# AdrianPerezHerrero/HDP-GPC

Measured on AMD Instinct MI355X. Metric: GP log-lik evals/sec (NxK batch, T-point segments), higher is better.
Workload: dtype f64; 1 GPU; BASELINE configs[1]: synthetic 2048 segments x 8 clusters, T=128, fp64, irregular segment grids (per-pair Gram + Cholesky + score); segments=2048, segments_per_gpu=2048, clusters=8, T=128

## Files before the change

hdpgpc_amd/csrc/hgp_internal.hpp:

```cpp
#pragma once
#include <hip/hip_runtime.h>
#include <stdint.h>
#include <stdlib.h>

#include <vector>

#include "../../include/hdpgpc_hip.h"

constexpr int WAVES = 4;

static inline int launch_status() {
  hipError_t e = hipGetLastError();
  return e == hipSuccess ? 0 : 1000 + (int)e;
}

static inline int nb_for(int n) {
  int nb = (n + 15) / 16;
  nb = (nb + 1) & ~1;
  return nb < 2 ? 2 : nb;
}

static inline bool env_on(const char* name) {
  const char* v = getenv(name);
  return v && v[0] && v[0] != '0';
}

constexpr double PAIRS_CUT = 55.45177444479562;
constexpr int PAIRS_FB_CAP = 65536;

static inline int acc_grid_for(int nb) { return nb > 8 ? 256 : 512; }

struct hgp_pairs_plan {
  int T, K, TP, NB;
  std::vector<double> theta;
  std::vector<int32_t> perm;
  std::vector<int> grp_beg, grp_end;
  std::vector<double> grp_ell;
  double *d_theta, *d_scal, *d_A, *d_S, *d_Z, *d_Kinv, *d_P, *d_Q, *d_Mp, *d_ap, *d_xb;
  int32_t* d_perm;
  bool coop = false;
  double* d_escr = nullptr;
  int32_t* d_eflags = nullptr;
  int nscr = 0;
  long escr_stride = 0;
  double acc_tol = 1e-9;
  double* d_Lop = nullptr;
  double* d_LTop = nullptr;
  double* d_Dop = nullptr;
  double* d_Sop = nullptr;
  double* d_mu = nullptr;
  int32_t* d_acc_list = nullptr;
  double* d_sscr = nullptr;
  int32_t* d_fb = nullptr;
  int score_out = 0;
};

int hgp_internal_acc_prep(hgp_pairs_plan* p, const double* mean, hipStream_t st);
int hgp_internal_pairs_acc(const hgp_pairs_plan* p, const double* x, const double* y, int N, int Ts, const double* first_noise,
                           const int32_t* sel, double* out_quad, double* out_logdet, int32_t* out_info, hipStream_t st);
size_t hgp_internal_acc_bytes(int TP, int K, size_t* sizes );

int hgp_internal_loglik_rows_b(const double* q, int N, int K, int B, double* out, hipStream_t st);
int hgp_internal_assign_b(const double* fmsg, const double* bmsg, int N, int K, int B, int64_t* labels, double* last_log, hipStream_t st);
// ... 50 lines not shown
```

hdpgpc_amd/csrc/hgp_kernels.hip:

```cpp
#include <hip/hip_runtime.h>
#include <math.h>
#include <stdint.h>
#include <string.h>

#include <algorithm>
#include <mutex>
#include <new>
#include <vector>

#include "../../include/hdpgpc_hip.h"
#include "hgp_internal.hpp"
#include "tile_f64.hpp"

using namespace hgp;

namespace {

__global__ void k_gram_rbf(const double* __restrict__ x, int nx, const double* __restrict__ y, int ny, double c,
                           double ell, double noise, int one_arg, double* __restrict__ K) {
  size_t idx = (size_t)blockIdx.x * blockDim.x + threadIdx.x;
  if (idx >= (size_t)nx * ny) return;
  int i = (int)(idx / ny), j = (int)(idx % ny);
  double u = x[i] / ell - (one_arg ? x[j] : y[j]) / ell;
  double v = c * exp(-0.5 * (u * u));
  if (one_arg && i == j) v = c + noise;
  K[idx] = v;
}

__global__ void k_mfma_probe(const double* __restrict__ A, const double* __restrict__ B, double* __restrict__ C) {
  const int lane = threadIdx.x & 63, g = lane >> 4, c = lane & 15;
  d4 acc = (d4){0.0, 0.0, 0.0, 0.0};
#pragma unroll
  for (int s = 0; s < 4; ++s) acc = mfma(A[c * 16 + 4 * s + g], B[(4 * s + g) * 16 + c], acc);
// ... 44 lines not shown
    add_diag<NB>(U, a.jitter_rel * fmax(dm, F64_EPS), T, lane);
  }
  PivotAcc pa;
  pa.init();
  wave_factor<NB, 0>(U, R, scr, nullptr, nullptr, lane, pa, A, T, T);
#pragma unroll
  for (int I = 0; I < NB; ++I)
#pragma unroll
    for (int J = I + 1; J < NB; ++J) {
      const int ln = launder(lane);
#pragma unroll
      for (int r = 0; r < 4; ++r) {
        int i = 16 * I + (ln >> 4) + 4 * r, j = 16 * J + (ln & 15);
        if (i < T && j < T) A[(size_t)i * T + j] = 0.0;
      }
    }
  if (lane == 0) {
    if (a.info) a.info[m] = pa.info;
    if (a.logdet) a.logdet[m] = pa.logdet();
  }
}

template <int NB>
__global__ __launch_bounds__(64 * WAVES) void k_wave_inv(PotrfArgs a) {
  __shared__ __attribute__((aligned(16))) double scr_all[WAVES * DIAG_SCR];
  const int wave = threadIdx.x >> 6, lane = threadIdx.x & 63;
  const int g = lane >> 4, c = lane & 15;
  const int w = blockIdx.x * WAVES + wave;
  const int m = w / NB, Jc = w % NB;
  const int T = a.T;
  if (m >= a.b || 16 * Jc >= T) return;
  double* scr = scr_all + wave * DIAG_SCR;
  const double* A = a.A + (size_t)m * T * T;
  d4 U[NB * (NB + 1) / 2];
  d4 R[NB];
  if (a.symmetric) load_upper_only<NB>(U, A, T, T, lane);
  else if constexpr (NB <= 6) load_sym_upper_burst<NB>(U, A, T, T, lane, scr);
  else load_sym_upper<NB>(U, A, T, T, lane, scr);
  {
    double sh = a.add;
    if (a.jitter_rel != 0.0) sh += a.jitter_rel * fmax(diag_abs_mean<NB>(U, T, lane, a.add), F64_EPS);
    if (sh != 0.0) add_diag<NB>(U, sh, T, lane);
  }
#pragma unroll
  for (int K = 0; K < NB; ++K)
#pragma unroll
    for (int r = 0; r < 4; ++r) R[K][r] = (K == Jc && g + 4 * r == c) ? 1.0 : 0.0;
  PivotAcc pa;
  pa.init();
  wave_factor<NB, 1>(U, R, scr, nullptr, nullptr, lane, pa, nullptr, 0, T);
  double* Z = a.Linv + (size_t)m * T * T;
#pragma unroll
  for (int K = 0; K < NB; ++K)
#pragma unroll
    for (int r = 0; r < 4; ++r) {
      const int i = 16 * K + g + 4 * r, j = 16 * Jc + c;
      if (i < T && j < T) Z[(size_t)i * T + j] = (K >= Jc) ? R[K][r] : 0.0;
    }
  if (a.inv_info && Jc == 0 && lane == 0 && a.info) a.info[m] = pa.info;
}

template <int NB>
void launch_wave_inv(const PotrfArgs& a, hipStream_t st) {
  const int waves = a.b * NB;
  hipLaunchKernelGGL(k_wave_inv<NB>, dim3((waves + WAVES - 1) / WAVES), dim3(64 * WAVES), 0, st, a);
}

struct ScoreArgs {
  const double* Y;
  int ldy;
  const double* mean;
  long mean_stride;
  const double* Sigma;
  long sigma_stride;
  int T;
  int ld_sigma;
  const int32_t* item_mat;
  const int32_t* item_mean;
  const double* item_add;
  const int32_t* item_off;
  const int32_t* item_cnt;
  int n_items;
// ... 275 lines not shown
#pragma unroll
      for (int s = 0; s < 4; ++s) {
        const int row = 16 * I + c, col = 16 * I + 4 * s + g;
        wv[s] = (row < T && col < T) ? Z[(size_t)row * T + col] : ((row == col) ? 1.0 : 0.0);
      }
      d4 z = (d4){0.0, 0.0, 0.0, 0.0};
#pragma unroll
      for (int s = 0; s < 4; ++s) z = mfma_sub(wv[s], acc0[s], z);
      Zc[I] = z;
    }
  }
  const bool bad = info && info[m] != 0;
#pragma unroll
  for (int I = 0; I < NB; ++I) {
#pragma unroll
    for (int r = 0; r < 4; ++r) {
      const int row = 16 * I + g + 4 * r, col = 16 * Kc + c;
      if (row < T && col < T && I != Kc) Z[(size_t)row * T + col] = bad ? __builtin_nan("") : ((I > Kc) ? Zc[I][r] : 0.0);
    }
  }
}

template <int NB>
__global__ __launch_bounds__(64 * WAVES) void k_coop_inv(PotrfArgs a) {
  using C = Coop<NB>;
  extern __shared__ __attribute__((aligned(16))) double smem[];
  double* rowbuf = smem;
  double* Rbuf = rowbuf + NB * 256;
  double* Wbuf = Rbuf + NB * 256;
  double* scr = Wbuf + 256;
  double* red = scr + DIAG_SCR;
  const int wave = __builtin_amdgcn_readfirstlane(threadIdx.x >> 6), lane = threadIdx.x & 63;
  const int g = lane >> 4, c = lane & 15;
  const int m = blockIdx.x, Jc = blockIdx.y;
  const int T = a.T;
  if (16 * Jc >= T) return;
  const double* A = a.A + (size_t)m * T * T;
  d4 U[C::NT];
  coop_load_sym_upper<NB>(U, A, T, T, wave, lane, rowbuf + wave * DIAG_SCR);
  __syncthreads();
  {
    double sh = a.add;
    if (a.jitter_rel != 0.0) {
      const double dm = coop_diag_abs_mean<NB>(U, T, wave, lane, a.add, red);
      sh += a.jitter_rel * fmax(dm, F64_EPS);
    }
    if (sh != 0.0) coop_add_diag<NB>(U, sh, T, wave, lane);
  }
  for (int K = wave; K < NB; K += WAVES) {
    d4 v;
#pragma unroll
    for (int r = 0; r < 4; ++r) v[r] = (K == Jc && g + 4 * r == c) ? 1.0 : 0.0;
    lds_tile_store(Rbuf, K, lane, v);
  }
  __syncthreads();
  PivotAcc pa;
  pa.init();
  coop_factor<NB, true>(U, rowbuf, Rbuf, Wbuf, scr, wave, lane, pa, nullptr, 0, T);
  double* Z = a.Linv + (size_t)m * T * T;
  for (int K = wave; K < NB; K += WAVES) {
    const d4 z = lds_tile_load(Rbuf, K, lane);
#pragma unroll
    for (int r = 0; r < 4; ++r) {
      const int i = 16 * K + g + 4 * r, j = 16 * Jc + c;
      if (i < T && j < T) Z[(size_t)i * T + j] = (K >= Jc) ? z[r] : 0.0;
    }
  }
  if (a.inv_info && Jc == 0) {
    int info;
    (void)coop_logdet_info(pa, wave, lane, red, reinterpret_cast<int*>(red + 8), info);
    if (threadIdx.x == 0 && a.info) a.info[m] = info;
  }
}

}

int hgp_internal_ensure_dynamic_lds(const void* fn, size_t bytes) {
  static std::mutex mu;
  static std::vector<std::pair<const void*, int>> done;
  int dv = 0;
  if (hipGetDevice(&dv) != hipSuccess) return launch_status();
  std::lock_guard<std::mutex> lk(mu);
  for (const auto& d : done)
    if (d.first == fn && d.second == dv) return 0;
  const hipError_t e = hipFuncSetAttribute(fn, hipFuncAttributeMaxDynamicSharedMemorySize, (int)bytes);
  if (e != hipSuccess) return 1000 + (int)e;
  done.emplace_back(fn, dv);
  return 0;
}

namespace {

template <int NB>
int launch_coop_score(const ScoreArgs& a, hipStream_t st) {
  const size_t lds = sizeof(double) * Coop<NB>::LDS_DOUBLES;
// ... 22 lines not shown
  if (int rc_ = hgp_internal_ensure_dynamic_lds(reinterpret_cast<const void*>(&k_coop_inv<NB>), lds)) return rc_;
  hipLaunchKernelGGL(k_coop_inv<NB>, dim3(a.b, NB), dim3(64 * WAVES), lds, st, a);
  return launch_status();
}

struct GemmArgs {
  const double* A;
  const double* B;
  double* C;
  int M, N, Kd, lda, ldb, ldc;
  long sA, sB, sC;
  double alpha, beta;
  int tA, tB;
  int nb2 = 1;
  long sA2 = 0, sB2 = 0, sC2 = 0;
  const double* D = nullptr;
  int ldd = 0;
  long sD = 0;
  int boff = 0;
  int triA = 0;
};

template <int TRIP>
__global__ __launch_bounds__(64 * WAVES) void k_gemm(GemmArgs a) {
  const int wave = threadIdx.x >> 6, lane = threadIdx.x & 63;
  const int g = lane >> 4, c = lane & 15;
  const int ntn = (a.N + 15) / 16, ntm = (a.M + 15) / 16;
  const int tile = blockIdx.x * WAVES + wave;
  if (tile >= ntm * ntn) return;
  const int ti = tile / ntn, tj = tile % ntn;
  const int by = (int)blockIdx.y + a.boff;
  const int b1 = by / a.nb2, b2 = by % a.nb2;
  const double* A = a.A + (size_t)b1 * a.sA + (size_t)b2 * a.sA2;
  const double* B = a.B + (size_t)b1 * a.sB + (size_t)b2 * a.sB2;
  double* C = a.C + (size_t)b1 * a.sC + (size_t)b2 * a.sC2;
  d4 acc = (d4){0.0, 0.0, 0.0, 0.0};
  const int row = 16 * ti + c, col = 16 * tj + c;
  int nk = (a.Kd + 3) / 4;
  if (a.triA && !a.tA) nk = min(nk, 4 * (ti + 1));
  for (int k0 = 0; k0 < nk; k0 += TRIP) {
    double av[TRIP], bv[TRIP];
#pragma unroll
    for (int u = 0; u < TRIP; ++u) {
      const int k = 4 * (k0 + u) + g;
      av[u] = 0.0;
      bv[u] = 0.0;
      if (k < a.Kd) {
        if (row < a.M) av[u] = a.tA ? A[(size_t)k * a.lda + row] : A[(size_t)row * a.lda + k];
        if (col < a.N) bv[u] = a.tB ? B[(size_t)col * a.ldb + k] : B[(size_t)k * a.ldb + col];
      }
    }
#pragma unroll
    for (int u = 0; u < TRIP; ++u) acc = mfma(av[u], bv[u], acc);
  }
#pragma unroll
  for (int r = 0; r < 4; ++r) {
    const int i = 16 * ti + g + 4 * r;
    if (i < a.M && col < a.N) {
      double v = a.alpha * acc[r];
      if (a.beta != 0.0)
        v += a.beta * (a.D ? a.D[(size_t)b1 * a.sD + (size_t)i * a.ldd + col] : C[(size_t)i * a.ldc + col]);
      C[(size_t)i * a.ldc + col] = v;
    }
  }
}

__global__ __launch_bounds__(64 * WAVES) void k_gemm22(GemmArgs a) {
  const int wave = threadIdx.x >> 6, lane = threadIdx.x & 63;
  const int g = lane >> 4, c = lane & 15;
  const int ntn = a.N / 32, ntm = a.M / 32;
  const int tile = blockIdx.x * WAVES + wave;
  if (tile >= ntm * ntn) return;
  const int ti = tile / ntn, tj = tile % ntn;
  const int by = (int)blockIdx.y + a.boff;
  const int b1 = by / a.nb2, b2 = by % a.nb2;
  const double* A = a.A + (size_t)b1 * a.sA + (size_t)b2 * a.sA2 + (size_t)(32 * ti + c) * a.lda + g;
  const double* B = a.B + (size_t)b1 * a.sB + (size_t)b2 * a.sB2 + (size_t)g * a.ldb + 32 * tj + c;
  double* C = a.C + (size_t)b1 * a.sC + (size_t)b2 * a.sC2;
  d4 acc[2][2];
#pragma unroll
  for (int i = 0; i < 2; ++i)
#pragma unroll
    for (int j = 0; j < 2; ++j) acc[i][j] = (d4){0.0, 0.0, 0.0, 0.0};
  int nk = a.Kd / 4;
  if (a.triA) nk = min(nk, 8 * (ti + 1));
  constexpr int TR = 8;
  for (int k0 = 0; k0 < nk; k0 += TR) {
// ... 847 lines not shown
      const int oi = redi[tid + w];
      if (ov > red[tid] || (ov == red[tid] && oi < redi[tid])) {
        red[tid] = ov;
        redi[tid] = oi;
      }
    }
    __syncthreads();
  }
  if (tid == 0) first[t] = (any_nan || redi[0] >= K * K) ? 0 : redi[0];
}

struct PrepArgs {
  const double* xb;
  const double* mean;
  const double* Sigma;
  int T, TP, K;
  const double* theta;
  double* scal;
  double* A;
  double* S;
  double* xb_copy;
};

__global__ __launch_bounds__(256) void k_prep_build(PrepArgs a) {
  __shared__ double red[256];
  __shared__ int redi[256];
  const int k = blockIdx.x, tid = threadIdx.x;
  const int T = a.T, TP = a.TP;
  const double* Sg = a.Sigma + (size_t)k * T * T;
  const double c = a.theta[3 * k], ell = a.theta[3 * k + 1], noise = a.theta[3 * k + 2];
  double s_abs = 0.0, s_sgn = 0.0;
  for (int i = tid; i < T; i += 256) {
    double d = Sg[(size_t)i * T + i];
    s_abs += fabs(d);
    s_sgn += d;
  }
  red[tid] = s_abs;
  __syncthreads();
  for (int o = 128; o > 0; o >>= 1) {
    if (tid < o) red[tid] += red[tid + o];
    __syncthreads();
  }
  const double mean_abs = red[0] / T;
  __syncthreads();
  red[tid] = s_sgn;
  __syncthreads();
  for (int o = 128; o > 0; o >>= 1) {
    if (tid < o) red[tid] += red[tid + o];
    __syncthreads();
  }
  const double mS = red[0] / T;
  int bad = 0;
  for (int i = tid; i < T; i += 256) {
    double d = Sg[(size_t)i * T + i];
    if (!(fabs(d - mS) <= 1e-8 + 1e-5 * fabs(mS))) bad = 1;
  }
  redi[tid] = bad;
  __syncthreads();
  for (int o = 128; o > 0; o >>= 1) {
    if (tid < o) redi[tid] |= redi[tid + o];
    __syncthreads();
  }
  const double jit = 1e-4 * fmax(mean_abs, F64_EPS);
  if (tid == 0 && blockIdx.y == 0) {
    double* sc = a.scal + 8 * k;
    sc[0] = c;
    sc[1] = ell;
    sc[2] = noise;
    sc[3] = redi[0] ? 0.0 : 1.0;
    sc[4] = mS;
    sc[5] = jit;
    sc[6] = 0.0;
  }
  if (k == 0 && blockIdx.y == 0)
    for (int i = tid; i < TP; i += 256) a.xb_copy[i] = (i < T) ? a.xb[i] : 0.0;
  double* Ak = a.A + (size_t)k * TP * TP;
  double* Sk = a.S + (size_t)k * TP * TP;
  for (int idx = blockIdx.y * 256 + tid; idx < TP * TP; idx += gridDim.y * 256) {
    int i = idx / TP, j = idx % TP;
    double av, sv = 0.0;
    if (i < T && j < T) {
      double u = a.xb[i] / ell - a.xb[j] / ell;
      av = c * exp(-0.5 * (u * u));
      if (i == j) av += jit;
      sv = 0.5 * (Sg[(size_t)i * T + j] + Sg[(size_t)j * T + i]);
    } else {
      av = (i == j) ? 1.0 : 0.0;
    }
    Ak[idx] = av;
    Sk[idx] = sv;
  }
}

struct PrepFinalArgs {
  const double* Q;
  const double* Kinv;
  const double* mean;
  double* scal;
  int T, TP;
  double* Mp;
  double* ap;
  int interleave;
  int32_t* fb;
};

__global__ __launch_bounds__(256) void k_prep_final(PrepFinalArgs a) {
  const int k = blockIdx.x, tid = threadIdx.x;
  if (a.fb && k == 0 && blockIdx.y == 0 && tid == 0) {
    a.fb[0] = 0;
    a.fb[1 + PAIRS_FB_CAP] = 0;
  }
  const int T = a.T, TP = a.TP;
  const double c = a.scal[8 * k];
  const double* Q = a.Q + (size_t)k * TP * TP;
  const double* Ki = a.Kinv + (size_t)k * TP * TP;
  double* Mp = a.Mp + (size_t)k * TP * TP;
  __shared__ double tq[32][33], tk[32][33];
  const int NHh = (TP / 16) / 2, nt = TP / 32;
  const int tx = tid & 31, ty = tid >> 5;
  for (int t = blockIdx.y; t < nt * nt; t += gridDim.y) {
    const int bi = t / nt, bj = t % nt;
    __syncthreads();
#pragma unroll
    for (int r = 0; r < 4; ++r) {
      const int y = ty + 8 * r;
      tq[y][tx] = Q[(size_t)(32 * bj + y) * TP + 32 * bi + tx];
      tk[y][tx] = Ki[(size_t)(32 * bj + y) * TP + 32 * bi + tx];
    }
    __syncthreads();
#pragma unroll
    for (int r = 0; r < 4; ++r) {
      const int y = ty + 8 * r;
      const int i = 32 * bi + y, j = 32 * bj + tx;
      double v = 0.0;
      if (i < T && j < T)
        v = (c * c) * (0.5 * (Q[(size_t)i * TP + j] + tq[tx][y]) - 0.5 * (Ki[(size_t)i * TP + j] + tk[tx][y]));
      int jp = j;
      if (a.interleave) {
        const int hh = j / (16 * NHh), tl = (j / 16) % NHh, cc = j % 16;
        const int loc = (tl < 2 * (NHh / 2)) ? 32 * (tl / 2) + 2 * cc + (tl & 1) : 16 * (NHh - 1) + cc;
        jp = 16 * NHh * hh + loc;
      }
      Mp[(size_t)i * TP + jp] = v;
    }
  }
  const double* mu = a.mean + (size_t)k * T;
  __shared__ double red[256];
  double rmax = 0.0;
  for (int i = blockIdx.y * 256 + tid; i < TP; i += gridDim.y * 256) {
    double s = 0.0, rs = 0.0;
    if (i < T) {
#pragma unroll 8
      for (int j = 0; j < T; ++j) {
        const double kij = Ki[(size_t)j * TP + i];
        s = fma(kij, mu[j], s);
        rs += fabs(kij);
      }
    }
    a.ap[(size_t)k * TP + i] = c * s;
    rmax = fmax(rmax, rs);
  }
  red[tid] = rmax;
  __syncthreads();
  for (int o = 128; o > 0; o >>= 1) {
    if (tid < o) red[tid] = fmax(red[tid], red[tid + o]);
    __syncthreads();
  }
  if (tid == 0) atomicMax(reinterpret_cast<unsigned long long*>(a.scal + 8 * k + 6), (unsigned long long)__double_as_longlong(red[0]));
}

}

#ifdef HGP_STAMPS
unsigned long long* hgp_internal_stamp_dev = nullptr;
#endif

static int tp_for(int n) {
  if (n <= HGP_MAX_T_WAVE) return 16 * nb_for(n);
  return n <= 192 ? 192 : 256;
}

static size_t plan_bytes(int T, int Ts_max, int K, size_t* offs ) {
  const size_t TP = (size_t)tp_for(std::max(T, Ts_max));
  const size_t mat = (size_t)K * TP * TP * sizeof(double);
  size_t o = 0;
  auto take = [&](size_t bytes) {
    size_t at = o;
    o += (bytes + 255) & ~(size_t)255;
    return at;
  };
  size_t tmp[24] = {0};
// ... 97 lines not shown
  return launch_status();
}

size_t hgp_pairs_plan_device_bytes(int T, int Ts_max, int K) {
  if (T <= 0 || Ts_max <= 0 || K <= 0) return 0;
  return plan_bytes(T, Ts_max, K, nullptr);
}

int hgp_pairs_plan_create(hgp_pairs_plan** plan, int T, int Ts_max, int K, const double* theta_host, void* dev_buf,
                          size_t dev_bytes) {
  if (!plan || !theta_host || !dev_buf || T <= 0 || Ts_max <= 0 || K <= 0) return -1;
  if (T > HGP_MAX_T_COOP || Ts_max > HGP_MAX_T_COOP) return -2;
  size_t offs[24];
  if (dev_bytes < plan_bytes(T, Ts_max, K, offs)) return -1;
  for (int k = 0; k < K; ++k)
    if (!(theta_host[3 * k] > 0.0) || !(theta_host[3 * k + 1] > 0.0)) return -1;
  hgp_pairs_plan* p = new (std::nothrow) hgp_pairs_plan();
  if (!p) return -1;
  p->T = T;
  p->K = K;
  p->TP = tp_for(std::max(T, Ts_max));
  p->NB = p->TP / 16;
  p->coop = p->TP > HGP_MAX_T_WAVE;
  p->theta.assign(theta_host, theta_host + 3 * (size_t)K);
  p->perm.resize(K);
  for (int k = 0; k < K; ++k) p->perm[k] = k;
  std::stable_sort(p->perm.begin(), p->perm.end(),
                   [&](int a, int b) { return p->theta[3 * a + 1] < p->theta[3 * b + 1]; });
  for (int i = 0; i < K;) {
    int j = i;
    double ell = p->theta[3 * p->perm[i] + 1];
    while (j < K && p->theta[3 * p->perm[j] + 1] == ell) ++j;
    p->grp_beg.push_back(i);
    p->grp_end.push_back(j);
    p->grp_ell.push_back(ell);
    i = j;
  }
  char* base = (char*)dev_buf;
  p->d_theta = (double*)(base + offs[0]);
  p->d_scal = (double*)(base + offs[1]);
  p->d_A = (double*)(base + offs[2]);
  p->d_S = (double*)(base + offs[3]);
  p->d_Z = (double*)(base + offs[4]);
  p->d_Kinv = (double*)(base + offs[5]);
  p->d_P = (double*)(base + offs[6]);
  p->d_Q = (double*)(base + offs[7]);
// ... 24 lines not shown
      delete p;
      return 1000 + (int)hipGetLastError();
    }
  }
  if (hipMemcpy(p->d_theta, p->theta.data(), sizeof(double) * 3 * K, hipMemcpyHostToDevice) != hipSuccess ||
      hipMemcpy(p->d_perm, p->perm.data(), sizeof(int32_t) * K, hipMemcpyHostToDevice) != hipSuccess) {
    delete p;
    return 1000 + (int)hipGetLastError();
  }
  *plan = p;
  return 0;
}

void hgp_pairs_plan_destroy(hgp_pairs_plan* plan) { delete plan; }

const double* hgp_pairs_plan_scalars(const hgp_pairs_plan* plan) { return plan ? plan->d_scal : nullptr; }

int hgp_pairs_plan_update(hgp_pairs_plan* p, const double* x_basis, const double* mean, const double* Sigma,
                          int32_t* info, void* stream) {
  if (!p || !x_basis || !mean || !Sigma) return -1;
  hipStream_t st = (hipStream_t)stream;
  const int K = p->K, T = p->T, TP = p->TP;
  PrepArgs pa{x_basis, mean, Sigma, T, TP, K, p->d_theta, p->d_scal, p->d_A, p->d_S, p->d_xb};
  hipLaunchKernelGGL(k_prep_build, dim3(K, 8), dim3(256), 0, st, pa);
  PotrfArgs fa{p->d_A, TP, K, 0.0, 0.0, p->d_Z, nullptr, info};
  fa.inv_info = 1;
  fa.symmetric = 1;
  switch (p->NB) {
    case 2: launch_wave_inv<2>(fa, st); break;
    case 4: launch_wave_inv<4>(fa, st); break;
    case 6: launch_wave_inv<6>(fa, st); break;
    case 8:
      launch_coop_inv_only<8>(fa, st);
      break;
    case 12: launch_coop_potrf<12>(fa, st); break;
    default: launch_coop_potrf<16>(fa, st); break;
  }
  const long sm = (long)TP * TP;
  GemmArgs g1{p->d_Z, p->d_Z, p->d_Kinv, TP, TP, TP, TP, TP, TP, sm, sm, sm, 1.0, 0.0, 1, 0};
  GemmArgs g2{p->d_S, p->d_Kinv, p->d_P, TP, TP, TP, TP, TP, TP, sm, sm, sm, 1.0, 0.0, 0, 0};
  GemmArgs g3{p->d_Kinv, p->d_P, p->d_Q, TP, TP, TP, TP, TP, TP, sm, sm, sm, 1.0, 0.0, 0, 0};
  launch_gemm(g1, K, st);
  launch_gemm(g2, K, st);
  launch_gemm(g3, K, st);
  PrepFinalArgs fin{p->d_Q, p->d_Kinv, mean, p->d_scal, T, TP, p->d_Mp, p->d_ap, p->coop ? 0 : 1, p->d_fb};
  hipLaunchKernelGGL(k_prep_final, dim3(K, 8), dim3(256), 0, st, fin);
  if (p->d_eflags && p->nscr > 0 && hipMemsetAsync(p->d_eflags, 0, (p->nscr + 1) * sizeof(int32_t), st) != hipSuccess) return launch_status();
  int rc = hgp_internal_acc_prep(p, mean, st);
  return rc ? rc : launch_status();
}

int hgp_pairs_plan_set_accuracy(hgp_pairs_plan* p, double tol) {
  if (!p || tol != tol) return -1;
  p->acc_tol = tol;
  return 0;
}

int hgp_pairs_plan_set_score_output(hgp_pairs_plan* p, int on) {
  if (!p) return -1;
  p->score_out = on ? 1 : 0;
  return 0;
}

int hgp_loglik_pairs_f64(const hgp_pairs_plan* p, const double* x, const double* y, int N, int Ts,
                         const double* first_noise, const int32_t* sel, double* out_quad, double* out_logdet,
                         int32_t* out_info, void* stream) {
  if (N == 0) return 0;
  if (!p || !x || !y || !out_quad || N < 0 || Ts <= 0) return -1;
  if (Ts > HGP_MAX_T_COOP) return -2;
  if (Ts > p->TP) return -2;
// ... 250 lines not shown
```

hdpgpc_amd/csrc/hgp_pairs_acc.hip:

```cpp
#include <hip/hip_runtime.h>
#include <math.h>
#include <stdint.h>

#include "hgp_internal.hpp"
#include "tile_f64.hpp"

using namespace hgp;

namespace {

__host__ __device__ constexpr int ntl(int NB) { return NB * (NB - 1) / 2; }
__host__ __device__ constexpr int tl(int K, int Kp) { return K * (K - 1) / 2 + Kp; }

__global__ void k_acc_flags(double* scal, int K, double tol, int32_t* acc_list) {
  if (threadIdx.x != 0 || blockIdx.x != 0) return;
  int n = 0;
  for (int k = 0; k < K; ++k) {
    const double ck = scal[8 * k] * scal[8 * k + 6];
    const double bound = F64_EPS * ck * ck;
    const bool flag = (tol == 0.0) || (tol > 0.0 && !(bound <= tol));
    scal[8 * k + 7] = flag ? 1.0 : 0.0;
    if (flag) acc_list[1 + n++] = k;
  }
  acc_list[0] = n;
}

template <int NB>
__global__ __launch_bounds__(64) void k_acc_factor(double* A, int TP, const double* scal, int32_t* info) {
  __shared__ __attribute__((aligned(16))) double scr[DIAG_SCR];
  const int k = blockIdx.x, lane = threadIdx.x;
  if (scal[8 * k + 7] == 0.0) return;
  double* Ak = A + (size_t)k * TP * TP;
  d4 U[NB * (NB + 1) / 2];
  d4 R[NB];
  load_upper_only<NB>(U, Ak, TP, TP, lane);
  PivotAcc pa;
  pa.init();
  wave_factor<NB, 0>(U, R, scr, nullptr, nullptr, lane, pa, Ak, TP, TP);
  if (lane == 0 && info && pa.info != 0) info[k] = pa.info;
}

struct AccPrepArgs {
  const double* L;
  const double* S;
  const double* mean;
  const double* scal;
  int T, TP, NB;
  double* Lop;
  double* LTop;
  double* Dop;
  double* Sop;
  double* mu;
};

__global__ __launch_bounds__(256) void k_acc_prep(AccPrepArgs a) {
  const int k = blockIdx.x;
  if (a.scal[8 * k + 7] == 0.0) return;
  const int lane = threadIdx.x & 63, g = lane >> 4, c = lane & 15;
  const int wv = blockIdx.y * 4 + (threadIdx.x >> 6), nwv = gridDim.y * 4;
  const int NB = a.NB, TP = a.TP;
  const double* L = a.L + (size_t)k * TP * TP;
  const double* S = a.S + (size_t)k * TP * TP;
  const int nl = ntl(NB);
  double* Lop = a.Lop + (size_t)k * nl * 256;
  double* LTop = a.LTop + (size_t)k * nl * 256;
  double* Dop = a.Dop + (size_t)k * 4 * NB * 256;
  double* Sop = a.Sop + (size_t)k * NB * NB * 256;
  if (blockIdx.y == 0)
    for (int i = threadIdx.x; i < TP; i += 256) a.mu[(size_t)k * TP + i] = (i < a.T) ? a.mean[(size_t)k * a.T + i] : 0.0;
  const int items = nl + NB + NB * NB;
  for (int it = wv; it < items; it += nwv) {
    if (it < nl) {
      int Kb = 1;
      while (tl(Kb + 1, 0) <= it) ++Kb;
      const int Kp = it - tl(Kb, 0);
      d4 lo, lt;
#pragma unroll
      for (int s = 0; s < 4; ++s) {
        lo[s] = L[(size_t)(16 * Kb + c) * TP + 16 * Kp + 4 * s + g];
        lt[s] = L[(size_t)(16 * Kb + 4 * s + g) * TP + 16 * Kp + c];
      }
      *reinterpret_cast<d4*>(Lop + ((size_t)it * 64 + lane) * 4) = lo;
      *reinterpret_cast<d4*>(LTop + ((size_t)it * 64 + lane) * 4) = lt;
    } else if (it < nl + NB) {
      const int Kb = it - nl;
      const double* D = L + (size_t)(16 * Kb) * TP + 16 * Kb;
      d4 a1, a2, a1t, a2t;
#pragma unroll
      for (int r = 0; r < 4; ++r) {
        const double* B = D + (size_t)(4 * r) * TP + 4 * r;
        const double l00 = B[0], l10 = B[TP], l11 = B[TP + 1], l20 = B[2 * TP], l21 = B[2 * TP + 1], l22 = B[2 * TP + 2],
                     l30 = B[3 * (size_t)TP], l31 = B[3 * (size_t)TP + 1], l32 = B[3 * (size_t)TP + 2], l33 = B[3 * (size_t)TP + 3];
        double w[4][4];
#pragma unroll
        for (int i = 0; i < 4; ++i)
#pragma unroll
          for (int j = 0; j < 4; ++j) w[i][j] = 0.0;
        const double r0 = 1.0 / l00, r1 = 1.0 / l11, r2 = 1.0 / l22, r3 = 1.0 / l33;
        w[0][0] = r0;
        w[1][0] = -(l10 * w[0][0]) * r1;
        w[2][0] = -(l20 * w[0][0] + l21 * w[1][0]) * r2;
        w[3][0] = -(l30 * w[0][0] + l31 * w[1][0] + l32 * w[2][0]) * r3;
        w[1][1] = r1;
        w[2][1] = -(l21 * w[1][1]) * r2;
        w[3][1] = -(l31 * w[1][1] + l32 * w[2][1]) * r3;
        w[2][2] = r2;
        w[3][2] = -(l32 * w[2][2]) * r3;
        w[3][3] = r3;
        const int ci = c & 3;
        double wf = 0.0, wt = 0.0;
#pragma unroll
        for (int i = 0; i < 4; ++i)
#pragma unroll
          for (int j = 0; j < 4; ++j) {
            if (i == ci && j == g) wf = w[i][j];
            if (i == g && j == ci) wt = w[i][j];
          }
        const bool mine = (c >> 2) == r;
        a1[r] = mine ? wf : 0.0;
        a1t[r] = mine ? wt : 0.0;
        a2[r] = (c >= 4 * r + 4) ? D[(size_t)c * TP + 4 * r + g] : 0.0;
        a2t[r] = (c < 4 * r) ? D[(size_t)(4 * r + g) * TP + c] : 0.0;
      }
      *reinterpret_cast<d4*>(Dop + ((size_t)(0 * NB + Kb) * 64 + lane) * 4) = a1;
      *reinterpret_cast<d4*>(Dop + ((size_t)(1 * NB + Kb) * 64 + lane) * 4) = a2;
      *reinterpret_cast<d4*>(Dop + ((size_t)(2 * NB + Kb) * 64 + lane) * 4) = a1t;
      *reinterpret_cast<d4*>(Dop + ((size_t)(3 * NB + Kb) * 64 + lane) * 4) = a2t;
    } else {
      const int t = it - nl - NB, Kb = t / NB, Kp = t % NB;
      d4 so;
#pragma unroll
      for (int s = 0; s < 4; ++s) so[s] = S[(size_t)(16 * Kp + 4 * s + g) * TP + 16 * Kb + c];
      *reinterpret_cast<d4*>(Sop + ((size_t)t * 64 + lane) * 4) = so;
    }
  }
}

struct AccArgs {
  const double* x;
  const double* y;
  int N, Ts;
  const double* xb;
  int T;
  const double* scal;
  const double* mu;
  const double* Lop;
  const double* LTop;
  const double* Dop;
  const double* Sop;
  const int32_t* acc_list;
  const double* first_noise;
  const int32_t* sel;
  int K;
  double* out_quad;
  double* out_logdet;
  int32_t* out_info;
  double* sscr;
  double score_add;
  int score_on;
// ... 280 lines not shown
```

Measured before the change: 15.49 million evals/s.

## Fuse plan-update stages into one cooperative kernel with grid syncs

The plan update used to issue a chain of separate kernels: build, inverse, three GEMMs, final, acc flags, acc factor and acc prep. The kernel bodies are now device functions, called in sequence from a single cooperative kernel separated by grid.sync(). This applies when the plan is non-coop and K*NB blocks fit in the measured cooperative occupancy. The aim is to remove per-launch overhead and inter-kernel gaps. In exchange the GEMM phases run on a small fixed grid, every phase pays grid-wide barrier cost, and the eflags memset was dropped from the update path.

New measurement: 14.47 million evals/s. -6.6%, worse.

```diff
diff --git a/hdpgpc_amd/csrc/hgp_acc_prep.hpp b/hdpgpc_amd/csrc/hgp_acc_prep.hpp
--- /dev/null
+++ b/hdpgpc_amd/csrc/hgp_acc_prep.hpp
@@ -0,0 +1,132 @@
+#pragma once
+#include <hip/hip_runtime.h>
+#include <stdint.h>
+
+#include "tile_f64.hpp"
+
+namespace hgp {
+
+__host__ __device__ constexpr int ntl(int NB) { return NB * (NB - 1) / 2; }
+__host__ __device__ constexpr int tl(int K, int Kp) { return K * (K - 1) / 2 + Kp; }
+
+__device__ __forceinline__ void acc_flags_body(double* scal, int K, double tol, int32_t* acc_list) {
+  int n = 0;
+  for (int k = 0; k < K; ++k) {
+    const double ck = scal[8 * k] * scal[8 * k + 6];
+    const double bound = F64_EPS * ck * ck;
+    const bool flag = (tol == 0.0) || (tol > 0.0 && !(bound <= tol));
+    scal[8 * k + 7] = flag ? 1.0 : 0.0;
+    if (flag) acc_list[1 + n++] = k;
+  }
+  acc_list[0] = n;
+}
+
+template <int NB>
+__device__ __forceinline__ void acc_factor_body(double* A, int TP, const double* scal, int32_t* info, int k, int lane, double* scr) {
+  if (scal[8 * k + 7] == 0.0) return;
+  double* Ak = A + (size_t)k * TP * TP;
+  d4 U[NB * (NB + 1) / 2];
+  d4 R[NB];
+  load_upper_only<NB>(U, Ak, TP, TP, lane);
+  PivotAcc pa;
+  pa.init();
+  wave_factor<NB, 0>(U, R, scr, nullptr, nullptr, lane, pa, Ak, TP, TP);
+  if (lane == 0 && info && pa.info != 0) info[k] = pa.info;
+}
+
+struct AccPrepArgs {
+  const double* L;
+  const double* S;
+  const double* mean;
+  const double* scal;
+  int T, TP, NB;
+  double* Lop;
+  double* LTop;
+  double* Dop;
+  double* Sop;
+  double* mu;
+};
+
+__device__ __forceinline__ void acc_prep_body(const AccPrepArgs& a, int k, int by, int ny, int tid) {
+  if (a.scal[8 * k + 7] == 0.0) return;
+  const int lane = tid & 63, g = lane >> 4, c = lane & 15;
+  const int wv = by * 4 + (tid >> 6), nwv = ny * 4;
+  const int NB = a.NB, TP = a.TP;
+  const double* L = a.L + (size_t)k * TP * TP;
+  const double* S = a.S + (size_t)k * TP * TP;
+  const int nl = ntl(NB);
+  double* Lop = a.Lop + (size_t)k * nl * 256;
+  double* LTop = a.LTop + (size_t)k * nl * 256;
+  double* Dop = a.Dop + (size_t)k * 4 * NB * 256;
+  double* Sop = a.Sop + (size_t)k * NB * NB * 256;
+  if (by == 0)
+    for (int i = tid; i < TP; i += 256) a.mu[(size_t)k * TP + i] = (i < a.T) ? a.mean[(size_t)k * a.T + i] : 0.0;
+  const int items = nl + NB + NB * NB;
+  for (int it = wv; it < items; it += nwv) {
+    if (it < nl) {
+      int Kb = 1;
+      while (tl(Kb + 1, 0) <= it) ++Kb;
+      const int Kp = it - tl(Kb, 0);
+      d4 lo, lt;
+#pragma unroll
+      for (int s = 0; s < 4; ++s) {
+        lo[s] = L[(size_t)(16 * Kb + c) * TP + 16 * Kp + 4 * s + g];
+        lt[s] = L[(size_t)(16 * Kb + 4 * s + g) * TP + 16 * Kp + c];
+      }
+      *reinterpret_cast<d4*>(Lop + ((size_t)it * 64 + lane) * 4) = lo;
+      *reinterpret_cast<d4*>(LTop + ((size_t)it * 64 + lane) * 4) = lt;
+    } else if (it < nl + NB) {
+      const int Kb = it - nl;
+      const double* D = L + (size_t)(16 * Kb) * TP + 16 * Kb;
+      d4 a1, a2, a1t, a2t;
+#pragma unroll
+      for (int r = 0; r < 4; ++r) {
+        const double* B = D + (size_t)(4 * r) * TP + 4 * r;
+        const double l00 = B[0], l10 = B[TP], l11 = B[TP + 1], l20 = B[2 * TP], l21 = B[2 * TP + 1], l22 = B[2 * TP + 2],
+                     l30 = B[3 * (size_t)TP], l31 = B[3 * (size_t)TP + 1], l32 = B[3 * (size_t)TP + 2], l33 = B[3 * (size_t)TP + 3];
+        double w[4][4];
+#pragma unroll
+        for (int i = 0; i < 4; ++i)
+#pragma unroll
+          for (int j = 0; j < 4; ++j) w[i][j] = 0.0;
+        const double r0 = 1.0 / l00, r1 = 1.0 / l11, r2 = 1.0 / l22, r3 = 1.0 / l33;
+        w[0][0] = r0;
+        w[1][0] = -(l10 * w[0][0]) * r1;
+        w[2][0] = -(l20 * w[0][0] + l21 * w[1][0]) * r2;
+        w[3][0] = -(l30 * w[0][0] + l31 * w[1][0] + l32 * w[2][0]) * r3;
+        w[1][1] = r1;
+        w[2][1] = -(l21 * w[1][1]) * r2;
+        w[3][1] = -(l31 * w[1][1] + l32 * w[2][1]) * r3;
+        w[2][2] = r2;
+        w[3][2] = -(l32 * w[2][2]) * r3;
+        w[3][3] = r3;
+        const int ci = c & 3;
+        double wf = 0.0, wt = 0.0;
+#pragma unroll
+        for (int i = 0; i < 4; ++i)
+#pragma unroll
+          for (int j = 0; j < 4; ++j) {
+            if (i == ci && j == g) wf = w[i][j];
+            if (i == g && j == ci) wt = w[i][j];
+          }
+        const bool mine = (c >> 2) == r;
+        a1[r] = mine ? wf : 0.0;
+        a1t[r] = mine ? wt : 0.0;
+        a2[r] = (c >= 4 * r + 4) ? D[(size_t)c * TP + 4 * r + g] : 0.0;
+        a2t[r] = (c < 4 * r) ? D[(size_t)(4 * r + g) * TP + c] : 0.0;
+      }
+      *reinterpret_cast<d4*>(Dop + ((size_t)(0 * NB + Kb) * 64 + lane) * 4) = a1;
+      *reinterpret_cast<d4*>(Dop + ((size_t)(1 * NB + Kb) * 64 + lane) * 4) = a2;
+      *reinterpret_cast<d4*>(Dop + ((size_t)(2 * NB + Kb) * 64 + lane) * 4) = a1t;
+      *reinterpret_cast<d4*>(Dop + ((size_t)(3 * NB + Kb) * 64 + lane) * 4) = a2t;
+    } else {
+      const int t = it - nl - NB, Kb = t / NB, Kp = t % NB;
+      d4 so;
+#pragma unroll
+      for (int s = 0; s < 4; ++s) so[s] = S[(size_t)(16 * Kp + 4 * s + g) * TP + 16 * Kb + c];
+      *reinterpret_cast<d4*>(Sop + ((size_t)t * 64 + lane) * 4) = so;
+    }
+  }
+}
+
+}
diff --git a/hdpgpc_amd/csrc/hgp_internal.hpp b/hdpgpc_amd/csrc/hgp_internal.hpp
--- a/hdpgpc_amd/csrc/hgp_internal.hpp
+++ b/hdpgpc_amd/csrc/hgp_internal.hpp
@@ -39,6 +39,7 @@
   double *d_theta, *d_scal, *d_A, *d_S, *d_Z, *d_Kinv, *d_P, *d_Q, *d_Mp, *d_ap, *d_xb;
   int32_t* d_perm;
   bool coop = false;
+  int update_grid_max = 0;
   double* d_escr = nullptr;
   int32_t* d_eflags = nullptr;
   int nscr = 0;
diff --git a/hdpgpc_amd/csrc/hgp_kernels.hip b/hdpgpc_amd/csrc/hgp_kernels.hip
--- a/hdpgpc_amd/csrc/hgp_kernels.hip
+++ b/hdpgpc_amd/csrc/hgp_kernels.hip
@@ -1,3 +1,4 @@
+#include <hip/hip_cooperative_groups.h>
 #include <hip/hip_runtime.h>
 #include <math.h>
 #include <stdint.h>
@@ -9,6 +10,7 @@
 #include <vector>
 
 #include "../../include/hdpgpc_hip.h"
+#include "hgp_acc_prep.hpp"
 #include "hgp_internal.hpp"
 #include "tile_f64.hpp"
 
@@ -99,15 +101,11 @@
 }
 
 template <int NB>
-__global__ __launch_bounds__(64 * WAVES) void k_wave_inv(PotrfArgs a) {
-  __shared__ __attribute__((aligned(16))) double scr_all[WAVES * DIAG_SCR];
-  const int wave = threadIdx.x >> 6, lane = threadIdx.x & 63;
+__device__ __forceinline__ void wave_inv_body(const PotrfArgs& a, int w, int lane, double* scr) {
   const int g = lane >> 4, c = lane & 15;
-  const int w = blockIdx.x * WAVES + wave;
   const int m = w / NB, Jc = w % NB;
   const int T = a.T;
   if (m >= a.b || 16 * Jc >= T) return;
-  double* scr = scr_all + wave * DIAG_SCR;
   const double* A = a.A + (size_t)m * T * T;
   d4 U[NB * (NB + 1) / 2];
   d4 R[NB];
@@ -135,6 +133,13 @@
       if (i < T && j < T) Z[(size_t)i * T + j] = (K >= Jc) ? R[K][r] : 0.0;
     }
   if (a.inv_info && Jc == 0 && lane == 0 && a.info) a.info[m] = pa.info;
+}
+
+template <int NB>
+__global__ __launch_bounds__(64 * WAVES) void k_wave_inv(PotrfArgs a) {
+  __shared__ __attribute__((aligned(16))) double scr_all[WAVES * DIAG_SCR];
+  const int wave = threadIdx.x >> 6, lane = threadIdx.x & 63;
+  wave_inv_body<NB>(a, blockIdx.x * WAVES + wave, lane, scr_all + wave * DIAG_SCR);
 }
 
 template <int NB>
@@ -456,17 +461,15 @@
 }
 
 template <int NB>
-__global__ __launch_bounds__(64 * WAVES) void k_coop_inv(PotrfArgs a) {
+__device__ __forceinline__ void coop_inv_body(const PotrfArgs& a, int m, int Jc, int tid, double* smem) {
   using C = Coop<NB>;
-  extern __shared__ __attribute__((aligned(16))) double smem[];
   double* rowbuf = smem;
   double* Rbuf = rowbuf + NB * 256;
   double* Wbuf = Rbuf + NB * 256;
   double* scr = Wbuf + 256;
   double* red = scr + DIAG_SCR;
-  const int wave = __builtin_amdgcn_readfirstlane(threadIdx.x >> 6), lane = threadIdx.x & 63;
+  const int wave = __builtin_amdgcn_readfirstlane(tid >> 6), lane = tid & 63;
   const int g = lane >> 4, c = lane & 15;
-  const int m = blockIdx.x, Jc = blockIdx.y;
   const int T = a.T;
   if (16 * Jc >= T) return;
   const double* A = a.A + (size_t)m * T * T;
@@ -503,8 +506,14 @@
   if (a.inv_info && Jc == 0) {
     int info;
     (void)coop_logdet_info(pa, wave, lane, red, reinterpret_cast<int*>(red + 8), info);
-    if (threadIdx.x == 0 && a.info) a.info[m] = info;
-  }
+    if (tid == 0 && a.info) a.info[m] = info;
+  }
+}
+
+template <int NB>
+__global__ __launch_bounds__(64 * WAVES) void k_coop_inv(PotrfArgs a) {
+  extern __shared__ __attribute__((aligned(16))) double smem[];
+  coop_inv_body<NB>(a, blockIdx.x, blockIdx.y, threadIdx.x, smem);
 }
 
 }
@@ -573,14 +582,12 @@
 };
 
 template <int TRIP>
-__global__ __launch_bounds__(64 * WAVES) void k_gemm(GemmArgs a) {
-  const int wave = threadIdx.x >> 6, lane = threadIdx.x & 63;
+__device__ __forceinline__ void gemm_tile_body(const GemmArgs& a, int tile, int by, int lane) {
   const int g = lane >> 4, c = lane & 15;
   const int ntn = (a.N + 15) / 16, ntm = (a.M + 15) / 16;
-  const int tile = blockIdx.x * WAVES + wave;
   if (tile >= ntm * ntn) return;
   const int ti = tile / ntn, tj = tile % ntn;
-  const int by = (int)blockIdx.y + a.boff;
+  by += a.boff;
   const int b1 = by / a.nb2, b2 = by % a.nb2;
   const double* A = a.A + (size_t)b1 * a.sA + (size_t)b2 * a.sA2;
   const double* B = a.B + (size_t)b1 * a.sB + (size_t)b2 * a.sB2;
@@ -614,6 +621,12 @@
       C[(size_t)i * a.ldc + col] = v;
     }
   }
+}
+
+template <int TRIP>
+__global__ __launch_bounds__(64 * WAVES) void k_gemm(GemmArgs a) {
+  const int wave = threadIdx.x >> 6, lane = threadIdx.x & 63;
+  gemm_tile_body<TRIP>(a, blockIdx.x * WAVES + wave, (int)blockIdx.y, lane);
 }
 
 __global__ __launch_bounds__(64 * WAVES) void k_gemm22(GemmArgs a) {
@@ -1507,10 +1520,9 @@
   double* xb_copy;
 };
 
-__global__ __launch_bounds__(256) void k_prep_build(PrepArgs a) {
+__device__ __forceinline__ void prep_build_body(const PrepArgs& a, int k, int by, int ny, int tid) {
   __shared__ double red[256];
   __shared__ int redi[256];
-  const int k = blockIdx.x, tid = threadIdx.x;
   const int T = a.T, TP = a.TP;
   const double* Sg = a.Sigma + (size_t)k * T * T;
   const double c = a.theta[3 * k], ell = a.theta[3 * k + 1], noise = a.theta[3 * k + 2];
@@ -1547,7 +1559,7 @@
     __syncthreads();
   }
   const double jit = 1e-4 * fmax(mean_abs, F64_EPS);
-  if (tid == 0 && blockIdx.y == 0) {
+  if (tid == 0 && by == 0) {
     double* sc = a.scal + 8 * k;
     sc[0] = c;
     sc[1] = ell;
@@ -1557,11 +1569,11 @@
     sc[5] = jit;
     sc[6] = 0.0;
   }
-  if (k == 0 && blockIdx.y == 0)
+  if (k == 0 && by == 0)
     for (int i = tid; i < TP; i += 256) a.xb_copy[i] = (i < T) ? a.xb[i] : 0.0;
   double* Ak = a.A + (size_t)k * TP * TP;
   double* Sk = a.S + (size_t)k * TP * TP;
-  for (int idx = blockIdx.y * 256 + tid; idx < TP * TP; idx += gridDim.y * 256) {
+  for (int idx = by * 256 + tid; idx < TP * TP; idx += ny * 256) {
     int i = idx / TP, j = idx % TP;
     double av, sv = 0.0;
     if (i < T && j < T) {
@@ -1576,6 +1588,8 @@
     Sk[idx] = sv;
   }
 }
+
+__global__ __launch_bounds__(256) void k_prep_build(PrepArgs a) { prep_build_body(a, blockIdx.x, blockIdx.y, gridDim.y, threadIdx.x); }
 
 struct PrepFinalArgs {
   const double* Q;
@@ -1589,9 +1603,8 @@
   int32_t* fb;
 };
 
-__global__ __launch_bounds__(256) void k_prep_final(PrepFinalArgs a) {
-  const int k = blockIdx.x, tid = threadIdx.x;
-  if (a.fb && k == 0 && blockIdx.y == 0 && tid == 0) {
+__device__ __forceinline__ void prep_final_body(const PrepFinalArgs& a, int k, int by, int ny, int tid) {
+  if (a.fb && k == 0 && by == 0 && tid == 0) {
     a.fb[0] = 0;
     a.fb[1 + PAIRS_FB_CAP] = 0;
   }
@@ -1603,7 +1616,7 @@
   __shared__ double tq[32][33], tk[32][33];
   const int NHh = (TP / 16) / 2, nt = TP / 32;
   const int tx = tid & 31, ty = tid >> 5;
-  for (int t = blockIdx.y; t < nt * nt; t += gridDim.y) {
+  for (int t = by; t < nt * nt; t += ny) {
     const int bi = t / nt, bj = t % nt;
     __syncthreads();
 #pragma unroll
@@ -1632,7 +1645,7 @@
   const double* mu = a.mean + (size_t)k * T;
   __shared__ double red[256];
   double rmax = 0.0;
-  for (int i = blockIdx.y * 256 + tid; i < TP; i += gridDim.y * 256) {
+  for (int i = by * 256 + tid; i < TP; i += ny * 256) {
     double s = 0.0, rs = 0.0;
     if (i < T) {
 #pragma unroll 8
@@ -1652,6 +1665,83 @@
     __syncthreads();
   }
   if (tid == 0) atomicMax(reinterpret_cast<unsigned long long*>(a.scal + 8 * k + 6), (unsigned long long)__double_as_longlong(red[0]));
+}
+
+__global__ __launch_bounds__(256) void k_prep_final(PrepFinalArgs a) { prep_final_body(a, blockIdx.x, blockIdx.y, gridDim.y, threadIdx.x); }
+
+struct PlanUpdateArgs {
+  PrepArgs build;
+  PotrfArgs inv;
+  GemmArgs g1, g2, g3;
+  PrepFinalArgs fin;
+  double acc_tol;
+  int32_t* acc_list;
+  AccPrepArgs acc;
+};
+
+template <int TRIP, int NB>
+__device__ __forceinline__ void plan_gemm_phase(const GemmArgs& g, int k, int by, int wave, int lane) {
+  for (int tile = by * WAVES + wave; tile < NB * NB; tile += NB * WAVES) gemm_tile_body<TRIP>(g, tile, k, lane);
+}
+
+template <int NB>
+__global__ __launch_bounds__(64 * WAVES) void k_plan_update(PlanUpdateArgs a) {
+  constexpr int TRIP = (NB == 2) ? 8 : (NB == 8 ? 32 : 24);
+  extern __shared__ __attribute__((aligned(16))) double smem[];
+  namespace cg = cooperative_groups;
+  cg::grid_group grid = cg::this_grid();
+  const int k = blockIdx.x, by = blockIdx.y, tid = threadIdx.x;
+  const int wave = tid >> 6, lane = tid & 63;
+  prep_build_body(a.build, k, by, NB, tid);
+  grid.sync();
+  if constexpr (NB == 8) {
+    coop_inv_body<8>(a.inv, k, by, tid, smem);
+  } else {
+    if (wave == 0) wave_inv_body<NB>(a.inv, k * NB + by, lane, smem);
+  }
+  grid.sync();
+  plan_gemm_phase<TRIP, NB>(a.g1, k, by, wave, lane);
+  grid.sync();
+  plan_gemm_phase<TRIP, NB>(a.g2, k, by, wave, lane);
+  grid.sync();
+  plan_gemm_phase<TRIP, NB>(a.g3, k, by, wave, lane);
+  grid.sync();
+  prep_final_body(a.fin, k, by, NB, tid);
+  grid.sync();
+  if (k == 0 && by == 0 && tid == 0) acc_flags_body(a.fin.scal, a.build.K, a.acc_tol, a.acc_list);
+  grid.sync();
+  if (a.acc_list[0] == 0) return;
+  if (by == 0 && wave == 0) acc_factor_body<NB>(a.inv.A, a.inv.T, a.fin.scal, nullptr, k, lane, smem);
+  grid.sync();
+  acc_prep_body(a.acc, k, by, NB, tid);
+}
+
+template <int NB>
+constexpr size_t plan_update_lds() {
+  if constexpr (NB == 8) return sizeof(double) * Coop<8>::LDS_DOUBLES;
+  else return sizeof(double) * DIAG_SCR;
+}
+
+template <int NB>
+int plan_update_max_grid() {
+  int dev = 0, coop = 0, cus = 0, per_cu = 0;
+  if (hipGetDevice(&dev) != hipSuccess || hipDeviceGetAttribute(&coop, hipDeviceAttributeCooperativeLaunch, dev) != hipSuccess ||
+      hipDeviceGetAttribute(&cus, hipDeviceAttributeMultiprocessorCount, dev) != hipSuccess ||
+      hipOccupancyMaxActiveBlocksPerMultiprocessor(&per_cu, k_plan_update<NB>, 64 * WAVES, plan_update_lds<NB>()) != hipSuccess) {
+    (void)hipGetLastError();
+    return 0;
+  }
+  if (!coop || per_cu <= 0 || cus <= 0) return 0;
+  if (per_cu > 1) --per_cu;
+  return per_cu * cus;
+}
+
+template <int NB>
+int launch_plan_update(PlanUpdateArgs& a, int K, hipStream_t st) {
+  void* args[] = {&a};
+  const hipError_t e = hipLaunchCooperativeKernel(reinterpret_cast<const void*>(&k_plan_update<NB>), dim3(K, NB), dim3(64 * WAVES), args,
+                                                  (unsigned)plan_update_lds<NB>(), st);
+  return e == hipSuccess ? launch_status() : 1000 + (int)e;
 }
 
 }
@@ -1795,6 +1885,13 @@
   p->TP = tp_for(std::max(T, Ts_max));
   p->NB = p->TP / 16;
   p->coop = p->TP > HGP_MAX_T_WAVE;
+  switch (p->coop ? 0 : p->NB) {
+    case 2: p->update_grid_max = plan_update_max_grid<2>(); break;
+    case 4: p->update_grid_max = plan_update_max_grid<4>(); break;
+    case 6: p->update_grid_max = plan_update_max_grid<6>(); break;
+    case 8: p->update_grid_max = plan_update_max_grid<8>(); break;
+    default: break;
+  }
   p->theta.assign(theta_host, theta_host + 3 * (size_t)K);
   p->perm.resize(K);
   for (int k = 0; k < K; ++k) p->perm[k] = k;
@@ -1865,10 +1962,25 @@
   hipStream_t st = (hipStream_t)stream;
   const int K = p->K, T = p->T, TP = p->TP;
   PrepArgs pa{x_basis, mean, Sigma, T, TP, K, p->d_theta, p->d_scal, p->d_A, p->d_S, p->d_xb};
-  hipLaunchKernelGGL(k_prep_build, dim3(K, 8), dim3(256), 0, st, pa);
   PotrfArgs fa{p->d_A, TP, K, 0.0, 0.0, p->d_Z, nullptr, info};
   fa.inv_info = 1;
   fa.symmetric = 1;
+  const long sm = (long)TP * TP;
+  GemmArgs g1{p->d_Z, p->d_Z, p->d_Kinv, TP, TP, TP, TP, TP, TP, sm, sm, sm, 1.0, 0.0, 1, 0};
+  GemmArgs g2{p->d_S, p->d_Kinv, p->d_P, TP, TP, TP, TP, TP, TP, sm, sm, sm, 1.0, 0.0, 0, 0};
+  GemmArgs g3{p->d_Kinv, p->d_P, p->d_Q, TP, TP, TP, TP, TP, TP, sm, sm, sm, 1.0, 0.0, 0, 0};
+  PrepFinalArgs fin{p->d_Q, p->d_Kinv, mean, p->d_scal, T, TP, p->d_Mp, p->d_ap, p->coop ? 0 : 1, p->d_fb};
+  if (!p->coop && (long)K * p->NB <= (long)p->update_grid_max) {
+    PlanUpdateArgs ua{pa, fa, g1, g2, g3, fin, p->acc_tol, p->d_acc_list,
+                      AccPrepArgs{p->d_A, p->d_S, mean, p->d_scal, T, TP, p->NB, p->d_Lop, p->d_LTop, p->d_Dop, p->d_Sop, p->d_mu}};
+    switch (p->NB) {
+      case 2: return launch_plan_update<2>(ua, K, st);
+      case 4: return launch_plan_update<4>(ua, K, st);
+      case 6: return launch_plan_update<6>(ua, K, st);
+      default: return launch_plan_update<8>(ua, K, st);
+    }
+  }
+  hipLaunchKernelGGL(k_prep_build, dim3(K, 8), dim3(256), 0, st, pa);
   switch (p->NB) {
     case 2: launch_wave_inv<2>(fa, st); break;
     case 4: launch_wave_inv<4>(fa, st); break;
@@ -1879,16 +1991,10 @@
     case 12: launch_coop_potrf<12>(fa, st); break;
     default: launch_coop_potrf<16>(fa, st); break;
   }
-  const long sm = (long)TP * TP;
-  GemmArgs g1{p->d_Z, p->d_Z, p->d_Kinv, TP, TP, TP, TP, TP, TP, sm, sm, sm, 1.0, 0.0, 1, 0};
-  GemmArgs g2{p->d_S, p->d_Kinv, p->d_P, TP, TP, TP, TP, TP, TP, sm, sm, sm, 1.0, 0.0, 0, 0};
-  GemmArgs g3{p->d_Kinv, p->d_P, p->d_Q, TP, TP, TP, TP, TP, TP, sm, sm, sm, 1.0, 0.0, 0, 0};
   launch_gemm(g1, K, st);
   launch_gemm(g2, K, st);
   launch_gemm(g3, K, st);
-  PrepFinalArgs fin{p->d_Q, p->d_Kinv, mean, p->d_scal, T, TP, p->d_Mp, p->d_ap, p->coop ? 0 : 1, p->d_fb};
   hipLaunchKernelGGL(k_prep_final, dim3(K, 8), dim3(256), 0, st, fin);
-  if (p->d_eflags && p->nscr > 0 && hipMemsetAsync(p->d_eflags, 0, (p->nscr + 1) * sizeof(int32_t), st) != hipSuccess) return launch_status();
   int rc = hgp_internal_acc_prep(p, mean, st);
   return rc ? rc : launch_status();
 }
diff --git a/hdpgpc_amd/csrc/hgp_pairs_acc.hip b/hdpgpc_amd/csrc/hgp_pairs_acc.hip
--- a/hdpgpc_amd/csrc/hgp_pairs_acc.hip
+++ b/hdpgpc_amd/csrc/hgp_pairs_acc.hip
@@ -2,6 +2,7 @@
 #include <math.h>
 #include <stdint.h>
 
+#include "hgp_acc_prep.hpp"
 #include "hgp_internal.hpp"
 #include "tile_f64.hpp"
 
@@ -9,132 +10,18 @@
 
 namespace {
 
-__host__ __device__ constexpr int ntl(int NB) { return NB * (NB - 1) / 2; }
-__host__ __device__ constexpr int tl(int K, int Kp) { return K * (K - 1) / 2 + Kp; }
-
 __global__ void k_acc_flags(double* scal, int K, double tol, int32_t* acc_list) {
   if (threadIdx.x != 0 || blockIdx.x != 0) return;
-  int n = 0;
-  for (int k = 0; k < K; ++k) {
-    const double ck = scal[8 * k] * scal[8 * k + 6];
-    const double bound = F64_EPS * ck * ck;
-    const bool flag = (tol == 0.0) || (tol > 0.0 && !(bound <= tol));
-    scal[8 * k + 7] = flag ? 1.0 : 0.0;
-    if (flag) acc_list[1 + n++] = k;
-  }
-  acc_list[0] = n;
+  acc_flags_body(scal, K, tol, acc_list);
 }
 
 template <int NB>
 __global__ __launch_bounds__(64) void k_acc_factor(double* A, int TP, const double* scal, int32_t* info) {
   __shared__ __attribute__((aligned(16))) double scr[DIAG_SCR];
-  const int k = blockIdx.x, lane = threadIdx.x;
-  if (scal[8 * k + 7] == 0.0) return;
-  double* Ak = A + (size_t)k * TP * TP;
-  d4 U[NB * (NB + 1) / 2];
-  d4 R[NB];
-  load_upper_only<NB>(U, Ak, TP, TP, lane);
-  PivotAcc pa;
-  pa.init();
-  wave_factor<NB, 0>(U, R, scr, nullptr, nullptr, lane, pa, Ak, TP, TP);
-  if (lane == 0 && info && pa.info != 0) info[k] = pa.info;
-}
-
-struct AccPrepArgs {
-  const double* L;
-  const double* S;
-  const double* mean;
-  const double* scal;
-  int T, TP, NB;
-  double* Lop;
-  double* LTop;
-  double* Dop;
-  double* Sop;
-  double* mu;
-};
-
-__global__ __launch_bounds__(256) void k_acc_prep(AccPrepArgs a) {
-  const int k = blockIdx.x;
-  if (a.scal[8 * k + 7] == 0.0) return;
-  const int lane = threadIdx.x & 63, g = lane >> 4, c = lane & 15;
-  const int wv = blockIdx.y * 4 + (threadIdx.x >> 6), nwv = gridDim.y * 4;
-  const int NB = a.NB, TP = a.TP;
-  const double* L = a.L + (size_t)k * TP * TP;
-  const double* S = a.S + (size_t)k * TP * TP;
-  const int nl = ntl(NB);
-  double* Lop = a.Lop + (size_t)k * nl * 256;
-  double* LTop = a.LTop + (size_t)k * nl * 256;
-  double* Dop = a.Dop + (size_t)k * 4 * NB * 256;
-  double* Sop = a.Sop + (size_t)k * NB * NB * 256;
-  if (blockIdx.y == 0)
-    for (int i = threadIdx.x; i < TP; i += 256) a.mu[(size_t)k * TP + i] = (i < a.T) ? a.mean[(size_t)k * a.T + i] : 0.0;
-  const int items = nl + NB + NB * NB;
-  for (int it = wv; it < items; it += nwv) {
-    if (it < nl) {
-      int Kb = 1;
-      while (tl(Kb + 1, 0) <= it) ++Kb;
-      const int Kp = it - tl(Kb, 0);
-      d4 lo, lt;
-#pragma unroll
-      for (int s = 0; s < 4; ++s) {
-        lo[s] = L[(size_t)(16 * Kb + c) * TP + 16 * Kp + 4 * s + g];
-        lt[s] = L[(size_t)(16 * Kb + 4 * s + g) * TP + 16 * Kp + c];
-      }
-      *reinterpret_cast<d4*>(Lop + ((size_t)it * 64 + lane) * 4) = lo;
-      *reinterpret_cast<d4*>(LTop + ((size_t)it * 64 + lane) * 4) = lt;
-    } else if (it < nl + NB) {
-      const int Kb = it - nl;
-      const double* D = L + (size_t)(16 * Kb) * TP + 16 * Kb;
-      d4 a1, a2, a1t, a2t;
-#pragma unroll
-      for (int r = 0; r < 4; ++r) {
-        const double* B = D + (size_t)(4 * r) * TP + 4 * r;
-        const double l00 = B[0], l10 = B[TP], l11 = B[TP + 1], l20 = B[2 * TP], l21 = B[2 * TP + 1], l22 = B[2 * TP + 2],
-                     l30 = B[3 * (size_t)TP], l31 = B[3 * (size_t)TP + 1], l32 = B[3 * (size_t)TP + 2], l33 = B[3 * (size_t)TP + 3];
-        double w[4][4];
-#pragma unroll
-        for (int i = 0; i < 4; ++i)
-#pragma unroll
-          for (int j = 0; j < 4; ++j) w[i][j] = 0.0;
-        const double r0 = 1.0 / l00, r1 = 1.0 / l11, r2 = 1.0 / l22, r3 = 1.0 / l33;
-        w[0][0] = r0;
-        w[1][0] = -(l10 * w[0][0]) * r1;
-        w[2][0] = -(l20 * w[0][0] + l21 * w[1][0]) * r2;
-        w[3][0] = -(l30 * w[0][0] + l31 * w[1][0] + l32 * w[2][0]) * r3;
-        w[1][1] = r1;
-        w[2][1] = -(l21 * w[1][1]) * r2;
-        w[3][1] = -(l31 * w[1][1] + l32 * w[2][1]) * r3;
-        w[2][2] = r2;
-        w[3][2] = -(l32 * w[2][2]) * r3;
-        w[3][3] = r3;
-        const int ci = c & 3;
-        double wf = 0.0, wt = 0.0;
-#pragma unroll
-        for (int i = 0; i < 4; ++i)
-#pragma unroll
-          for (int j = 0; j < 4; ++j) {
-            if (i == ci && j == g) wf = w[i][j];
-            if (i == g && j == ci) wt = w[i][j];
-          }
-        const bool mine = (c >> 2) == r;
-        a1[r] = mine ? wf : 0.0;
-        a1t[r] = mine ? wt : 0.0;
-        a2[r] = (c >= 4 * r + 4) ? D[(size_t)c * TP + 4 * r + g] : 0.0;
-        a2t[r] = (c < 4 * r) ? D[(size_t)(4 * r + g) * TP + c] : 0.0;
-      }
-      *reinterpret_cast<d4*>(Dop + ((size_t)(0 * NB + Kb) * 64 + lane) * 4) = a1;
-      *reinterpret_cast<d4*>(Dop + ((size_t)(1 * NB + Kb) * 64 + lane) * 4) = a2;
-      *reinterpret_cast<d4*>(Dop + ((size_t)(2 * NB + Kb) * 64 + lane) * 4) = a1t;
-      *reinterpret_cast<d4*>(Dop + ((size_t)(3 * NB + Kb) * 64 + lane) * 4) = a2t;
-    } else {
-      const int t = it - nl - NB, Kb = t / NB, Kp = t % NB;
-      d4 so;
-#pragma unroll
-      for (int s = 0; s < 4; ++s) so[s] = S[(size_t)(16 * Kp + 4 * s + g) * TP + 16 * Kb + c];
-      *reinterpret_cast<d4*>(Sop + ((size_t)t * 64 + lane) * 4) = so;
-    }
-  }
-}
+  acc_factor_body<NB>(A, TP, scal, info, blockIdx.x, threadIdx.x, scr);
+}
+
+__global__ __launch_bounds__(256) void k_acc_prep(AccPrepArgs a) { acc_prep_body(a, blockIdx.x, blockIdx.y, gridDim.y, threadIdx.x); }
 
 struct AccArgs {
   const double* x;
```
